# holo-routing/holo

Measured on AMD Instinct MI355X. Metric: full-SPF runs/sec on 100k-vertex synthetic LSDB, higher is better.
Workload: dtype u32; 1 GPU; isis-100k: IS-IS L2 100000 routers / 1000000 directed entries, metrics U[1,100], 64 concurrent SPF roots per GPU per step (BASELINE.json configs[2]); n_vertices=100000, n_entries=1000000, mask_words=1, outputs=dist u32 + hops u16 + flags u16 + first-hop mask u64 per (root,vertex), in HBM, steps_in_flight=4, gather=none

## Files before the change

holo_amd/build.py:

```python
from __future__ import annotations

import os
import shutil
import subprocess

HERE = os.path.dirname(os.path.abspath(__file__))
CSRC = os.path.join(HERE, "csrc")
LIB = os.path.join(HERE, "libholo_spf_hip.so")
SOURCES = ["spf_capi.hip", "hub_sort.hip"]
DEPS = ["spf_capi.hip", "spf_kernels.hip.h", "spf_repair.hip.h", "spf_lfa.hip.h", "spf_rlfa.hip.h", "spf_tilfa.hip.h", "graph_build.hip.h", "spf_multi.hip.h", "hub_sort.hip", "hub_sort.h", os.path.join("..", "..", "include", "holo_spf_hip.h")]


def hipcc_path() -> str:
    for cand in (shutil.which("hipcc"), "/opt/rocm/bin/hipcc"):
        if cand and os.path.exists(cand):
            return cand
    raise RuntimeError("hipcc not found: cannot build libholo_spf_hip.so")


def needs_build() -> bool:
    if not os.path.exists(LIB):
        return True
    t = os.path.getmtime(LIB)
    return any(os.path.getmtime(os.path.join(CSRC, d)) > t for d in DEPS)


def build_lib(force: bool = False, verbose: bool = False) -> str:
    if not force and not needs_build():
        return LIB
    flags = ["--offload-arch=gfx950", "-O3", "-std=c++17", "-fPIC", "-Wall", "-Wno-unused-function",
             "-mllvm", "-amdgpu-kernarg-preload-count=16"]
    flags += os.environ.get("HSPF_BUILD_DEFS", "").split()
    objs, procs = [], []
# ... 31 lines not shown
```

holo_amd/csrc/spf_capi.hip:

```cpp
#include "../../include/holo_spf_hip.h"
#include "spf_kernels.hip.h"
#include "spf_repair.hip.h"
#include "graph_build.hip.h"
#include "graph_patch.hip.h"
#include "hub_sort.h"
#include "spf_lfa.hip.h"
#include "spf_rlfa.hip.h"
#include "spf_tilfa.hip.h"

#include <algorithm>
#include <chrono>
#include <cstdio>
#include <cstdlib>
#include <cstring>
#include <atomic>
#include <condition_variable>
#include <deque>
#include <functional>
#include <mutex>
#include <thread>
#include <new>
#include <string>
#include <vector>

using namespace hspf;

namespace {

// ... 123 lines not shown
    g.out_ptr = d_out_ptr; g.out_dst = d_out_dst; g.out_w = d_out_w; g.out_fpos = d_out_fpos;
    for (int x = 0; x < 9; ++x) g.xcd_start[x] = xcd_start[x];
    g.unit_first = n_heavy_chunks ? d_unit_first : nullptr;
    g.n_heavy_units = n_heavy_chunks * 4u;
    for (int x = 0; x < 9; ++x) g.xcd_heavy[x] = xcd_heavy(x);
    g.giant_vtx = d_giant; g.giant_slice0 = d_giant + n_giant; g.n_giant = n_giant;
    return g;
  }
};

struct hspf_ctx {
  int device = 0;
  hipStream_t stream = nullptr;
  bool own_stream = true;
  std::string last_error;
  hipEvent_t ev[7] = {};
  DevBuf dist, hv, mask, lane_flags, changed, st64, stamp, hnb, kcnt, swcnt;
  uint32_t lean_head = 4, lean_passes = 16;
  uint32_t lean_dense_pct = 30;
  uint32_t lean_stay_pct = 10;
  uint32_t lean_dense_passes = 16;
  uint32_t lean_max_passes = 48;
  uint32_t lean_multi_min_wgs = 4096;
  DevBuf o_dist, o_hops, o_flags, o_mask, o_rank;
  DevBuf o_pack, pk_flag;
  char *h_stage = nullptr;
  size_t h_stage_cap = 0;
  hipEvent_t ev_stage[2] = {};
  DevBuf ex_list, ex_heap, ex_pos;
  DevBuf rp_rank;
  DevBuf dyn_part;
  DevBuf rp_trace;
  DevBuf rp_z, rp_ord, rp_work, rp_status;
  uint32_t *h_rp = nullptr; size_t h_rp_cap = 0;
  uint32_t est_rp_rounds = 6;
  uint32_t est_rp = 10;
  DevBuf pf_ptr, pf_vtx, pf_met, pf_org;
  bool pf_shadow_ok = false;
  uint32_t pf_shadow_nv = 0, pf_res_np = 0, pf_res_ne = 0;
  const void *pf_res_ptr = nullptr, *pf_res_vtx = nullptr, *pf_res_met = nullptr;
  DevBuf pack;
  uint32_t last_diff_count = 0;
  DevBuf evs_scr, evs_rec;
  DevBuf rlfa_key;
  DevBuf tilfa_key, tilfa_tw;
  DevBuf lfa_tab, lfa_scal;
// ... 523 lines not shown
    case HSPF_E_INTERNAL: return "internal invariant violated";
    case HSPF_E_NO_PACKED: return "results do not fit packed words";
    default: return "unknown error";
  }
}

const char *hspf_last_error(const hspf_ctx *ctx) { return ctx ? ctx->last_error.c_str() : ""; }

int hspf_init(int device_ordinal, hspf_ctx **out) {
  if (!out) return HSPF_E_INVAL;
  *out = nullptr;
  int n = 0;
  if (hipGetDeviceCount(&n) != hipSuccess || n <= 0) return HSPF_E_NODEV;
  if (device_ordinal < 0 || device_ordinal >= n) return HSPF_E_NODEV;
  hspf_ctx *ctx = new (std::nothrow) hspf_ctx();
  if (!ctx) return HSPF_E_NOMEM;
  ctx->device = device_ordinal;
  if (const char *v = getenv("HSPF_VARIANT")) ctx->variant = (uint32_t)strtoul(v, nullptr, 0);
  if (const char *v = getenv("HSPF_SINGLE_MAX_N")) ctx->single_max_n = (uint32_t)strtoul(v, nullptr, 0);
  if (const char *v = getenv("HSPF_DENSE_PASSES")) ctx->lean_dense_passes = std::min<uint32_t>(std::max<uint32_t>((uint32_t)strtoul(v, nullptr, 0), 1u), 32u);
  if (const char *v = getenv("HSPF_DENSE_PCT")) ctx->lean_dense_pct = (uint32_t)strtoul(v, nullptr, 0);
  if (const char *v = getenv("HSPF_DENSE_STAY_PCT")) ctx->lean_stay_pct = (uint32_t)strtoul(v, nullptr, 0);
  if (const char *v = getenv("HSPF_DENSE_MIN_WGS")) ctx->lean_multi_min_wgs = (uint32_t)strtoul(v, nullptr, 0);
  if (const char *v = getenv("HSPF_LEAN_HEAD")) ctx->lean_head = std::min<uint32_t>((uint32_t)strtoul(v, nullptr, 0), 60u);
  if (const char *v = getenv("HSPF_LV_MAX_ROOTS")) ctx->lv_max_roots = (uint32_t)strtoul(v, nullptr, 0);
  if (const char *v = getenv("HSPF_LV_MIN_N")) ctx->lv_min_n = (uint32_t)strtoul(v, nullptr, 0);
  if (const char *v = getenv("HSPF_XCD_MAX_ROOTS")) ctx->xcd_max_roots = std::min<uint32_t>((uint32_t)strtoul(v, nullptr, 0), XCD_MAX_ROOTS);
  if (const char *v = getenv("HSPF_XCD_ALWAYS")) ctx->xcd_always = strtoul(v, nullptr, 0) != 0;
  if (const char *v = getenv("HSPF_XCD_SKEW")) ctx->xcd_skew = atoi(v) != 0;
  if (const char *v = getenv("HSPF_XCD_TIMEOUT_MS")) ctx->xcd_timeout_ms = (uint32_t)strtoul(v, nullptr, 0);
  if (const char *v = getenv("HSPF_XCD_ROW_COST")) ctx->xcd_row_cost = (uint32_t)strtoul(v, nullptr, 0);
  if (const char *v = getenv("HSPF_UNIT_HEAVY_DEG")) ctx->unit_heavy_deg = (uint32_t)strtoul(v, nullptr, 0);
  if (const char *v = getenv("HSPF_HUB_DEG")) ctx->hub_deg = (uint32_t)strtoul(v, nullptr, 0);
  if (const char *v = getenv("HSPF_TW_HOST_MAX")) ctx->tw_host_max = strtoull(v, nullptr, 0);
  if (const char *v = getenv("HSPF_PATCH_FULL")) ctx->patch_full = atoi(v) != 0;
  if (const char *v = getenv("HSPF_ASYNC_LANES")) ctx->lanes_cfg = std::min<uint32_t>(std::max<uint32_t>((uint32_t)strtoul(v, nullptr, 0), 1u), 8u);
  if (hipSetDevice(device_ordinal) != hipSuccess) { delete ctx; return HSPF_E_NODEV; }
  if (hipStreamCreateWithFlags(&ctx->stream, hipStreamNonBlocking) != hipSuccess) { delete ctx; return HSPF_E_HIP; }
  for (auto &e : ctx->ev)
    if (hipEventCreate(&e) != hipSuccess) { delete ctx; return HSPF_E_HIP; }
  if (hipHostMalloc((void **)&ctx->h_changed, sizeof(int) * 256, hipHostMallocDefault) != hipSuccess) { delete ctx; return HSPF_E_NOMEM; }
  ctx->h_changed_cap = 256;
  if (hipHostMalloc((void **)&ctx->h_info, sizeof(BuildInfo), hipHostMallocDefault) != hipSuccess) { hspf_shutdown(ctx); return HSPF_E_NOMEM; }
  *out = ctx;
  return HSPF_OK;
}
// ... 892 lines not shown
  d_changed = (int *)ctx->changed.p;
  gd = g->dev();
  tabs = SlotTabs{d_up + w_ptr, d_up + w_vtx, d_up + w_base};
  if (row_map) od.row_map = d_up + w_map;
  ignore_ovl = (run_flags & HSPF_RUN_IGNORE_OVERLOAD) ? 1u : 0u;
  net_nh = (run_flags & HSPF_RUN_NET_NEXTHOPS) ? 1u : 0u;
  return HSPF_OK;
}

int Run::upload_block() {
  {
    uint32_t *h = ctx->h_up + (ctx->h_up_sel ? ctx->h_up_cap / 8 : 0);
    const uint32_t *prev = ctx->h_up + (ctx->h_up_sel ? 0 : ctx->h_up_cap / 8);
    std::fill(h, h + up_bytes / 4, 0u);
    std::fill(h + w_roots, h + w_roots + L, HSPF_NO_ROOT);
    std::copy(roots, roots + n_roots, h + w_roots);
    std::copy(tab_ptr.begin(), tab_ptr.end(), h + w_ptr);
    std::copy(tab_vtx.begin(), tab_vtx.end(), h + w_vtx);
    std::copy(tab_base.begin(), tab_base.end(), h + w_base);
    for (uint32_t r = 0; r < L; ++r) h[w_map + r] = (row_map && r < n_roots) ? row_map[r] : r;
    const FusedGraph fg{gd, tabs, d_kcnt, giant ? (uint32_t *)ctx->giant_part.p : (uint32_t *)nullptr,
                        (g->n_zero_rows && !g->hopcount_like) ? (uint32_t *)ctx->dyn_part.p : (uint32_t *)nullptr, L};
    memcpy(h + w_fg, &fg, sizeof(FusedGraph));
    st.dbg[2] = (uint32_t)std::chrono::duration_cast<std::chrono::microseconds>(std::chrono::steady_clock::now() - t_entry).count();
    const bool same = ctx->up_valid && ctx->up_len == up_bytes && memcmp(h, prev, up_bytes) == 0;
    if (!same) {
      HIPCHK(ctx, hipMemcpyAsync(d_up, h, up_bytes, hipMemcpyHostToDevice, s));
      ctx->up_valid = true; ctx->up_len = up_bytes; ctx->h_up_sel ^= 1;
    }
  }
  return HSPF_OK;
}

int Run::init_state() {
  d_st = (uint64_t *)ctx->st64.p;
  d_stamp = (uint32_t *)ctx->stamp.p;
  use_fw = !fused && !(ctx->variant & 64u) && (!g->hopcount_like || W <= 4);
  defer = use_fw && g->n_leaf != 0 && g->max_path_metric != HSPF_DIST_INF && !g->hopcount_like && g->n_zero_rows == 0;
  HIPCHK(ctx, hipEventRecord(ctx->ev[0], s));
  if (fused) {
  } else if (defer) {
    HIPCHK(ctx, hipMemsetAsync(d_lf, 0, (size_t)L * 4, s));
    const dim3 ig((unsigned)std::min<size_t>((rows / 64 + 3) / 4, 8192));
    switch (W) {
      case 1: hipLaunchKernelGGL(k_init_fw_state<1>, ig, dim3(256), 0, s, n, B, (const uint8_t *)g->d_leaf, d_dist, d_hv, d_mask); break;
      case 2: hipLaunchKernelGGL(k_init_fw_state<2>, ig, dim3(256), 0, s, n, B, (const uint8_t *)g->d_leaf, d_dist, d_hv, d_mask); break;
      case 4: hipLaunchKernelGGL(k_init_fw_state<4>, ig, dim3(256), 0, s, n, B, (const uint8_t *)g->d_leaf, d_dist, d_hv, d_mask); break;
// ... 117 lines not shown
      const bool zrows = dyn_parts;
      if (use_lean && zrows) st.dbg[0] |= 2u;
      if (dyn_parts && hipMemsetAsync(ctx->dyn_part.p, 0, (size_t)DYN_PARTS * L * 4, s) != hipSuccess) { ctx->last_error = "dyn partials"; return HSPF_E_HIP; }
      if (nar) hipLaunchKernelGGL((k_init_fused<uint32_t>), dim3((L + 3) / 4), dim3(256), 0, s, gd, (uint32_t *)d_st, d_stamp, (uint8_t *)ctx->hnb.p, d_roots, tabs, L, ns);
      else     hipLaunchKernelGGL((k_init_fused<uint64_t>), dim3((L + 3) / 4), dim3(256), 0, s, gd, d_st, d_stamp, (uint8_t *)ctx->hnb.p, d_roots, tabs, L, ns);
      uint32_t n_f = 0;
      const bool maxinf = g->max_path_metric == HSPF_DIST_INF;
      const bool plan_on = use_lean && !(ctx->variant & 524288u);
      const bool multi = ctx->lean_dense_passes > 1u && (uint64_t)fgrid.x * B >= ctx->lean_multi_min_wgs;
      const uint32_t per_launch = multi ? (uint32_t)std::min<uint64_t>(ctx->lean_dense_passes, ((1ull << 31) - 1u) / ((uint64_t)fgrid.x * B)) : 1u;
      const uint32_t plan_h = plan_on ? std::min(ctx->lean_head, 60u) : 0u;
      const uint32_t plan_P = plan_on ? std::min(std::max(ctx->lean_passes, 2u), std::min(ctx->lean_max_passes, 62u)) : 0u;
      const uint32_t plan_nd = plan_on ? (plan_P + per_launch - 1u) / per_launch : 0u;
      const uint64_t all_rows = (uint64_t)n * B;
      const uint32_t thr_enter = (uint32_t)std::min<uint64_t>(0xFFFFFFF0u, std::max<uint64_t>(1u, all_rows * ctx->lean_dense_pct / (100u * LEAN_SAMPLE)));
      const uint32_t thr_stay = ctx->lean_stay_pct == 0u ? 0u : (uint32_t)std::min<uint64_t>(0xFFFFFFF0u, std::max<uint64_t>(1u, all_rows * ctx->lean_stay_pct / (100u * LEAN_SAMPLE)));
      if (use_lean) {
        int e2 = ensure(ctx, ctx->swcnt, LEAN_CTL_WORDS * 4, false);
        if (e2) return e2;
      }
      uint32_t *d_ctl = (uint32_t *)ctx->swcnt.p;
      if (plan_on) ctx->est_fused = std::max(ctx->est_fused, plan_h + plan_nd + (ctx->est_seen ? 2u : 13u));
      ctx->est_seen = true;
      rb_ctl = plan_on ? d_ctl : nullptr;
      int r2 = run_phase(ctx->est_fused, pre_zeroed, [&](uint32_t sweep) {
#define HSPF_LAUNCH_FUSED2(ST_, MI_, CN_, UN_, stp_) hipLaunchKernelGGL((k_fused<ST_, MI_, CN_, UN_>), fgrid, dim3(256), 0, s, d_fg, d_changed, (int)sweep, d_stamp, (const uint8_t *)ctx->hnb.p, n, gd.in_ptr, gd.out_ptr, gd.vflags, stp_, d_roots, d_lf, net_nh, ignore_ovl, P, gd.in_src, gd.in_w, gd.out_dst, gd.e_in)
#define HSPF_LAUNCH_FUSED(ST_, MI_, CN_, stp_) do { if (units) HSPF_LAUNCH_FUSED2(ST_, MI_, CN_, true, stp_); else HSPF_LAUNCH_FUSED2(ST_, MI_, CN_, false, stp_); } while (0)
        const bool units = g->n_heavy_chunks != 0;
        if (use_lean) {
#define HSPF_LAUNCH_LEAN3(CN_, MD_, HD_, BM_, ZR_, grid_, pgr_, base_, thr_) hipLaunchKernelGGL((k_fused_lean<CN_, MD_, HD_, BM_, ZR_>), grid_, dim3(256), 0, s, d_fg, d_changed, (int)sweep, d_stamp, (const uint8_t *)ctx->hnb.p, n, (const uint32_t *)g->d_ell_so, (const uint32_t *)g->d_ell_w, (uint32_t *)d_st, (const uint32_t *)g->d_ell_od, d_roots, d_lf, net_nh, ignore_ovl, P, d_ctl, B, pgr_, base_, thr_)
#define HSPF_LAUNCH_LEAN2(CN_, MD_, HD_, BM_, grid_, pgr_, base_, thr_) do { if (zrows) HSPF_LAUNCH_LEAN3(CN_, MD_, HD_, BM_, true, grid_, pgr_, base_, thr_); else HSPF_LAUNCH_LEAN3(CN_, MD_, HD_, BM_, false, grid_, pgr_, base_, thr_); } while (0)
#define HSPF_LAUNCH_LEAN_C(MD_, HD_, grid_, pgr_, base_, thr_) do { if (count_rows) HSPF_LAUNCH_LEAN2(true, MD_, HD_, false, grid_, pgr_, base_, thr_); else HSPF_LAUNCH_LEAN2(false, MD_, HD_, false, grid_, pgr_, base_, thr_); } while (0)
#define HSPF_LAUNCH_LEAN_B(MD_, HD_, grid_, pgr_, base_, thr_) do { if (count_rows) HSPF_LAUNCH_LEAN2(true, MD_, HD_, true, grid_, pgr_, base_, thr_); else HSPF_LAUNCH_LEAN2(false, MD_, HD_, true, grid_, pgr_, base_, thr_); } while (0)
          const uint32_t bm_blocks = (n + (uint32_t)FVPB - 1u) / (uint32_t)FVPB;
          const bool bmaj = B >= 8u && 8ull * ((B + 7u) / 8u) * bm_blocks * per_launch < (1ull << 31);
          const dim3 bgrid(8u * ((B + 7u) / 8u) * bm_blocks);
          const PassGrid pg0{};
          if (sweep < plan_h) HSPF_LAUNCH_LEAN_C(0, true, fgrid, pg0, 0u, thr_enter);
          else if (sweep < plan_h + plan_nd) {
            const uint32_t base = (sweep - plan_h) * per_launch, np = std::min(per_launch, plan_P - base);
            if (bmaj) HSPF_LAUNCH_LEAN_B(1, false, dim3(bgrid.x * np), pass_grid(bgrid.x, bm_blocks), base, thr_stay);
            else      HSPF_LAUNCH_LEAN_C(1, false, dim3(fgrid.x * B * np), pass_grid(fgrid.x * B, fgrid.x), base, thr_stay);
          } else if (plan_on && sweep == plan_h + plan_nd) HSPF_LAUNCH_LEAN_C(2, false, fgrid, pg0, 0u, 0u);
          else HSPF_LAUNCH_LEAN_C(0, false, fgrid, pg0, 0u, 0u);
#undef HSPF_LAUNCH_LEAN_C
#undef HSPF_LAUNCH_LEAN_B
#undef HSPF_LAUNCH_LEAN2
#undef HSPF_LAUNCH_LEAN3
          return;
        }
        if (giant) {
          const dim3 ggrid(g->n_giant_slices, B);
#define HSPF_LAUNCH_GIANT(ST_, MI_, stp_) do { if (P.hc) hipLaunchKernelGGL((k_giant_part<ST_, MI_, true>), ggrid, dim3(256), 0, s, d_fg, (const int *)d_changed, (int)sweep, (const uint32_t *)d_stamp, n, (const ST_ *)stp_, (const uint32_t *)d_roots, net_nh, ignore_ovl, P); \
                                            else hipLaunchKernelGGL((k_giant_part<ST_, MI_, false>), ggrid, dim3(256), 0, s, d_fg, (const int *)d_changed, (int)sweep, (const uint32_t *)d_stamp, n, (const ST_ *)stp_, (const uint32_t *)d_roots, net_nh, ignore_ovl, P); } while (0)
          if (nar)         HSPF_LAUNCH_GIANT(uint32_t, false, (uint32_t *)d_st);
          else if (maxinf) HSPF_LAUNCH_GIANT(uint64_t, true, d_st);
          else             HSPF_LAUNCH_GIANT(uint64_t, false, d_st);
#undef HSPF_LAUNCH_GIANT
        }
        if (count_rows) {
          if (nar)         HSPF_LAUNCH_FUSED(uint32_t, false, true, (uint32_t *)d_st);
// ... 2 lines not shown
        } else {
          if (nar)         HSPF_LAUNCH_FUSED(uint32_t, false, false, (uint32_t *)d_st);
          else if (maxinf) HSPF_LAUNCH_FUSED(uint64_t, true, false, d_st);
          else             HSPF_LAUNCH_FUSED(uint64_t, false, false, d_st);
        }
#undef HSPF_LAUNCH_FUSED2
#undef HSPF_LAUNCH_FUSED
      }, n_f, [&]() {
        (void)hipEventRecord(ctx->ev[2], s);
        if (dyn_parts) hipLaunchKernelGGL(k_lf_reduce, dim3((L + 255) / 256), dim3(256), 0, s, d_lf, (const uint32_t *)ctx->dyn_part.p, L);
        const int rg = spec_fill ? (int)chunk_last : -1;
        emit_reset = rg >= 0;
        if (nar) hipLaunchKernelGGL((k_emit_fused<uint32_t>), dim3((n + 63) / 64, B), dim3(256), 0, s, n, n_roots, (uint32_t *)d_st, P, ode, ns, use_lean ? d_lf : (uint32_t *)nullptr, (const int *)d_changed, rg, fillw);
        else     hipLaunchKernelGGL((k_emit_fused<uint64_t>), dim3((n + 63) / 64, B), dim3(256), 0, s, n, n_roots, d_st, P, ode, ns, (uint32_t *)nullptr, (const int *)d_changed, rg, fillw);
        (void)hipEventRecord(ctx->ev[4], s);
        tail_done = true;
      });
      spec_fill = nullptr;
      if (r2) return r2;
      if (spec_done) ctx->prefill = hspf_ctx::Prefill{true, g->build_id, n, B, (uint32_t)esz, spec_nz, L, true, ns, fillw};
      ctx->est_fused = n_f + 1;
      st.n_relax_launches += n_f;
      if (count_rows) for (uint32_t i = 0; i < 256; ++i) st.rows_recomputed += ctx->h_lane_flags[L + i];
      if (plan_on) {
        const uint32_t *hc = ctx->h_lane_flags + L + 256;
        uint32_t trig = plan_h;
        for (uint32_t k = 0; k < plan_h; ++k) if (hc[LEAN_CTL_DUE + k * LEAN_CTL_STRIDE] == LEAN_SENTINEL) { trig = k; break; }
        uint32_t used = 0;
        for (uint32_t k = 0; k < plan_P; ++k) if (hc[LEAN_CTL_PCH + k * LEAN_CTL_STRIDE] != 0u) used = k + 1u;
        st.dbg[1] = (used & 0xFFu) | ((trig & 0xFFu) << 8) | ((plan_P & 0xFFu) << 16) | ((plan_h & 0x7Fu) << 24);
        const bool last_triggers = plan_h != 0u && hc[LEAN_CTL_DUE + (plan_h - 1u) * LEAN_CTL_STRIDE] != LEAN_SENTINEL && hc[LEAN_CTL_DUE + (plan_h - 1u) * LEAN_CTL_STRIDE] >= thr_enter;
        if (trig < plan_h) ctx->lean_head = std::max(trig, 1u);
        else if (plan_h != 0u && !last_triggers && used >= 2u) ctx->lean_head = std::min(plan_h + 1u, 60u);
        ctx->lean_passes = used >= plan_P ? std::min(ctx->lean_max_passes, plan_P + plan_P / 2u + 1u) : std::max(used + 1u, 2u);
      }
      return HSPF_OK;
    }

int Run::lv_run() {
      int r2;
      if ((r2 = ensure(ctx, ctx->stamp, (size_t)n_roots * n * 4))) return r2;
      uint32_t *a_stamp = (uint32_t *)ctx->stamp.p;
      hipError_t er = hipMemsetAsync(d_lf, 0, (size_t)L * 4, s);
      if (er == hipSuccess) er = hipMemsetAsync(d_st, 0xFF, (size_t)n_roots * n * 8, s);
      if (er == hipSuccess) er = hipMemsetAsync(a_stamp, 0, (size_t)n_roots * n * 4, s);
      if (er == hipSuccess && count_rows) er = hipMemsetAsync(d_kcnt, 0, 256 * 4, s);
// ... 725 lines not shown
    for (int c = 0; c < 3; ++c) {
      const uint32_t off = start[c], nr = start[c + 1] - start[c];
      if (nr == 0 || c == last_cls) continue;
      hspf_lane::Job job{g, std::vector<uint32_t>(proots.begin() + off, proots.begin() + off + nr), run_flags, U, 0,
                         std::vector<uint32_t>(dest.begin() + off, dest.begin() + off + nr), n_roots};
      cls_ticket[c] = lane_submit(ctx, std::move(job));
    }
  int rc_first = HSPF_OK;
  for (int c = 2; c >= 0; --c) {
    const uint32_t off = start[c], nr = start[c + 1] - start[c];
    if (nr == 0) continue;
    hspf_stats lane_st{};
    if (cls_ticket[c]) rc = lane_collect(ctx, cls_ticket[c], &lane_st);
    else rc = run_impl(ctx, g, proots.data() + off, nr, run_flags, &U, false, dest.data() + off, n_roots);
    if (rc) { if (!rc_first) rc_first = rc; continue; }
    const hspf_stats &p = cls_ticket[c] ? lane_st : ctx->stats;
    acc.n_roots += p.n_roots; acc.n_batches += p.n_batches; acc.n_relax_launches += p.n_relax_launches;
    acc.n_dag_launches += p.n_dag_launches; acc.n_exact_roots += p.n_exact_roots; acc.n_repaired_roots += p.n_repaired_roots; acc.repair_sweeps = std::max(acc.repair_sweeps, p.repair_sweeps); acc.repair_evals += p.repair_evals; acc.repair_groups += p.repair_groups; acc.ms_repair += p.ms_repair;
    acc.n_mask_words = std::max(acc.n_mask_words, p.n_mask_words);
    acc.ms_total += p.ms_total; acc.ms_relax += p.ms_relax; acc.ms_dag += p.ms_dag; acc.ms_finish += p.ms_finish;
    acc.state_bytes = std::max(acc.state_bytes, p.state_bytes); acc.narrow_overflow += p.narrow_overflow;
    acc.rows_recomputed += p.rows_recomputed;
    acc.dbg[0] |= p.dbg[0]; acc.dbg[1] = ((acc.dbg[1] | p.dbg[1]) & 0x80000000u) | ((acc.dbg[1] & 0x7FFFFFFFu) + (p.dbg[1] & 0x7FFFFFFFu));
    acc.dbg[2] += p.dbg[2]; acc.dbg[3] += p.dbg[3];
  }
  if (rc_first) return rc_first;
  if (!leaf_jobs.empty()) {
    const auto t_leaf = std::chrono::steady_clock::now();
    (void)hipSetDevice(ctx->device);
    if ((rc = ensure(ctx, ctx->leaf_jobs, leaf_jobs.size() * sizeof(LeafRootJob), false))) return rc;
    HIPCHK(ctx, hipMemcpyAsync(ctx->leaf_jobs.p, leaf_jobs.data(), leaf_jobs.size() * sizeof(LeafRootJob), hipMemcpyHostToDevice, s));
    hipLaunchKernelGGL(k_leaf_root_rows, dim3((n + 255u) / 256u, (uint32_t)leaf_jobs.size()), dim3(256), 0, s, n,
                       (const LeafRootJob *)ctx->leaf_jobs.p, (const uint32_t *)g->d_row_ptr[g->cur], (const uint32_t *)g->d_metric[g->cur], g->max_path_metric, W, U.dist, U.hops,
                       U.vflags_out, U.first_hop_mask);
    HIPCHK(ctx, hipGetLastError());
    HIPCHK(ctx, hipStreamSynchronize(s));
    acc.n_roots += (uint32_t)leaf_jobs.size();
    const float ms = std::chrono::duration<float, std::milli>(std::chrono::steady_clock::now() - t_leaf).count();
    acc.ms_total += ms; acc.ms_finish += ms;
  }
  if (side_by_side) {
    const float wall = std::chrono::duration<float, std::milli>(std::chrono::steady_clock::now() - t_cls).count();
    if (wall < acc.ms_total) {
      const float k = wall / acc.ms_total;
      acc.ms_total = wall; acc.ms_relax *= k; acc.ms_dag *= k; acc.ms_finish *= k;
    }
  }
// ... 87 lines not shown
}

int hspf_get_stats(const hspf_ctx *ctx, hspf_stats *out) {
  if (!ctx || !out) return HSPF_E_INVAL;
  *out = ctx->stats;
  return HSPF_OK;
}


static int lanes_ensure(hspf_ctx *ctx) {
  if (!ctx->lanes.empty()) return HSPF_OK;
  if (ctx->parent) { ctx->last_error = "asynchronous runs on a lane context"; return HSPF_E_INVAL; }
  (void)hipSetDevice(ctx->device);
  for (uint32_t i = 0; i < ctx->lanes_cfg; ++i) {
    hspf_lane *ln = new (std::nothrow) hspf_lane();
    if (!ln) { lanes_shutdown(ctx); return HSPF_E_NOMEM; }
    int rc = hspf_init(ctx->device, &ln->sub);
    if (rc == HSPF_OK) {
      hspf_ctx *c = ln->sub;
      c->parent = ctx;
      c->variant = ctx->variant; c->single_max_n = ctx->single_max_n; c->lv_max_roots = ctx->lv_max_roots; c->lv_min_n = ctx->lv_min_n; c->xcd_max_roots = ctx->xcd_max_roots; c->xcd_timeout_ms = ctx->xcd_timeout_ms; c->xcd_skew = ctx->xcd_skew; c->xcd_always = ctx->xcd_always;
      c->lean_dense_pct = ctx->lean_dense_pct; c->lean_stay_pct = ctx->lean_stay_pct; c->lean_dense_passes = ctx->lean_dense_passes;
      c->lean_head = ctx->lean_head; c->lean_passes = ctx->lean_passes; c->hub_deg = ctx->hub_deg; c->lean_multi_min_wgs = ctx->lean_multi_min_wgs;
      c->unit_heavy_deg = ctx->unit_heavy_deg; c->xcd_row_cost = ctx->xcd_row_cost;
    }
    if (rc != HSPF_OK) { if (ln->sub) hspf_shutdown(ln->sub); delete ln; lanes_shutdown(ctx); ctx->last_error = "could not create a lane context"; return rc; }
    for (auto &e : ln->stage_ev) if (hipEventCreateWithFlags(&e, hipEventDisableTiming) != hipSuccess) e = nullptr;
    if (!ctx->copy_stream && hipStreamCreateWithFlags(&ctx->copy_stream, hipStreamNonBlocking) != hipSuccess) ctx->copy_stream = nullptr;
    ctx->lanes.push_back(ln);
    ln->th = std::thread([ln, nl = ctx->lanes_cfg]() {
      for (;;) {
        std::unique_lock<std::mutex> lk(ln->mu);
        ln->cv.wait(lk, [&] { return !ln->jobs.empty() || ln->quit; });
        if (ln->jobs.empty()) return;
        hspf_lane::Job job = std::move(ln->jobs.front());
        ln->jobs.pop_front();
        ln->running = true;
        lk.unlock();
        ln->cv.notify_all();
        (void)hipSetDevice(ln->sub->device);
        hipEvent_t job_copy_ev = nullptr;
        const int rc = guarded(ln->sub, [&]() {
          if (job.packed) {
            hspf_ctx *par = ln->sub->parent;
            const size_t need = (size_t)8 * job.roots.size() * job.g->n;
            const uint64_t max_pairs = 1ull << 26;
// ... 815 lines not shown
```

holo_amd/csrc/spf_kernels.hip.h:

```cpp
#pragma once
#include <hip/hip_runtime.h>
#include <stdint.h>
#include <type_traits>

namespace hspf {

constexpr uint32_t INF = 0xFFFFFFFFu;
constexpr uint32_t SRC_NO_TRANSIT = 0x80000000u;
constexpr uint32_t SRC_LEAF = 0x40000000u;
constexpr uint32_t SRC_MASK = 0x3FFFFFFFu;

constexpr uint32_t HV_EPOCH_SHIFT = 16;
constexpr uint32_t HV_EPOCH_MAX = 0xFFFFu;

constexpr uint32_t LF_NEED_EXACT = 1u;
constexpr uint32_t LF_OVERFLOW = 2u;
constexpr uint32_t LF_DYN = 4u;

constexpr int WAVES_PER_BLOCK = 4;
constexpr int VPW = 4;
constexpr int VPB = WAVES_PER_BLOCK * VPW;

struct GraphDev {
  uint32_t n;
// ... 1095 lines not shown
  const uint32_t bx = bmaj ? (fpass >> 3) - fq * pgr.blocks : (MODE == 1 ? fpass - fq * pgr.blocks : blockIdx.x);
  const uint32_t pg = MODE == 1 ? pass_base + pidx : 0u;
  uint32_t pc2 = LEAN_SENTINEL, pc3 = LEAN_SENTINEL;
  if (MODE == 1 && thr != 0u && pg >= 2u && pg < 64u) {
    pc2 = ctl[LEAN_CTL_PCH + (pg - 2u) * LEAN_CTL_STRIDE];
    if (pg >= 3u) pc3 = ctl[LEAN_CTL_PCH + (pg - 3u) * LEAN_CTL_STRIDE];
  }
  const bool sampler = wave == 0u && (bmaj ? (bx & 7u) == 0u : ((bx >> 3) & 7u) == 0u);
  const uint32_t chunk = bmaj ? bx : xcd_chunk(gp->g.xcd_start, bx);
  if (MODE == 1 && min(pc2, pc3) < thr) {
    if (bx == 0u && batch == 0u && threadIdx.x == 0) changed[sweep] = 1;
    return;
  }
  if (chunk == 0xFFFFFFFFu || (bmaj && batch >= nbat)) return;
  const uint32_t wbeg = chunk * (uint32_t)FVPB + wave * (uint32_t)FVPW;
  if (wbeg >= n) return;
  uint32_t *A = act + (size_t)batch * n;
  const uint32_t cur = (uint32_t)sweep + 2u;
  const uint32_t vl = min(wbeg + min(lane, (uint32_t)VPW - 1u), n - 1);
  const uint32_t av = MODE == 0 ? A[vl] : cur;
  const uint32_t hb = hnb[(size_t)batch * n + vl] & (ignore_ovl ? ~RF_NT : ~0u);
  const uint32_t due4 = (uint32_t)__ballot(lane < (uint32_t)VPW && wbeg + lane < n && av >= cur);
  if (MODE == 0 && due4 == 0u) return;
  if (HEAD && sampler && lane == 0 && (uint32_t)sweep < 64u) atomicAdd(&ctl[LEAN_CTL_DUE + (uint32_t)sweep * LEAN_CTL_STRIDE], (uint32_t)__builtin_popcount(due4));
  ST *S = st + (size_t)batch * (n + 1u) * 64;
  const __amdgpu_buffer_rsrc_t rs = st_rsrc(S, (n + 1u) << 8);
  const uint32_t lane4 = lane * 4u;
  uint32_t sov[VPW], wk[VPW], od[VPW], oldq[VPW];
#pragma unroll
  for (int i = 0; i < VPW; ++i) {
    const uint32_t e = (min(wbeg + i, n) * 16u + (lane & 15u)) * 4u;
    sov[i] = *(const uint32_t *)((const char *)ell_so + e);
    wk[i] = *(const uint32_t *)((const char *)ell_w + e);
    od[i] = MODE == 1 ? 0u : *(const uint32_t *)((const char *)ell_od + e);
    oldq[i] = __builtin_amdgcn_raw_buffer_load_b32(rs, lane4, min(wbeg + i, n - 1) << 8, 0);
  }
  const uint32_t fast4 = (uint32_t)__ballot(lane < (uint32_t)VPW && hb == 0u) & due4;
  const uint32_t fasth4 = (uint32_t)__ballot(lane < (uint32_t)VPW && (hb & ~RF_ROOT) == RF_HNB) & due4;
  const uint32_t fastz4 = (!ZROWS || P.hc) ? 0u : ((uint32_t)__ballot(lane < (uint32_t)VPW && hb == RF_ZERO) & due4);
  const uint32_t root_slot = batch * 64 + lane;
  const __amdgpu_buffer_rsrc_t ra = st_rsrc(A, n * 4u);
  uint32_t info[VPW];
#pragma unroll
  for (int i = 0; i < VPW; ++i) {
    info[i] = rdlane(sov[i], 0) & 0xFFu;
    sov[i] &= ~0xFFu;
    wk[i] = (wk[i] << P.sh) + ((lane & 7u) << (P.sh - 3u));
    od[i] = lane < 16u ? od[i] : 0xFFFFFFFFu;
  }
  uint64_t any = 0ull;
  bool dyn = false;
  uint32_t n_done = 0, n_chg = 0;
  lean_group<COUNT, MODE, ZROWS>(gp, rs, ra, lane, lane4, wbeg, cur, P, roots, root_slot, net_nexthops, ignore_ovl, due4, fast4, fasth4, fastz4,
                          sov, wk, od, oldq, info, any, dyn, n_done, n_chg);
  if (MODE == 1) { if (bx == 0u && batch == 0u && threadIdx.x == 0) changed[sweep] = 1; }
  else if (any != 0ull && lane == 0) changed[sweep] = 1;
  if (COUNT && lane == 0) atomicAdd(&gp->rows_done[(blockIdx.x + wave) & 255u], n_done);
  if (MODE == 1 && sampler && lane == 0 && n_chg != 0u && pg < 64u) atomicAdd(&ctl[LEAN_CTL_PCH + pg * LEAN_CTL_STRIDE], n_chg);
  if (ZROWS && dyn) raise_dyn(gp, lane_flags, root_slot, blockIdx.x * 4u + wave);
}

constexpr int SINGLE_THREADS = 1024;
constexpr uint32_t SINGLE_MAX_N = 8192;
constexpr uint32_t SINGLE_MAX_E = 65536;
constexpr size_t SINGLE_LDS_MAX = 160 * 1024 - 64;

__device__ __forceinline__ void single_store_flags(uint32_t *lane_flags, uint32_t root_slot, uint32_t lf, int *word) {
  __syncthreads();
  if (threadIdx.x == 0) *word = 0;
  __syncthreads();
  if (lf) atomicOr(word, (int)lf);
  __syncthreads();
  if (threadIdx.x == 0) lane_flags[root_slot] = (uint32_t)*word;
}

struct SingleArgs {
  const FusedGraph *gp;
  const uint32_t *roots;
  FusedParams P;
  uint32_t net_nexthops, ignore_ovl, n_roots, count_rows, lds_links;
  uint32_t *lane_flags;
// ... 1866 lines not shown
```

Before: 157,700 spf_runs/s.

## Add compacting scan kernel for sparse lean sweeps with learned per-sweep plan

Adds k_lean_scan, where each block first ballots due and fast-path bits for 16 chunks of vertices, then has its four waves work only through the groups that have due rows. This cuts the wave launches and idle waves that the lean kernel spends on sparse sweeps. A host-side plan records per-sweep due counts from the sampler and picks the scan kernel on later runs for sweeps whose count falls below a threshold. The sampler atomic now fires in all MODE 0 launches, and the debug counters are packed, which adds some atomics and a different grid shape.

```diff
diff --git a/holo_amd/build.py b/holo_amd/build.py
--- a/holo_amd/build.py
+++ b/holo_amd/build.py
@@ -8,7 +8,7 @@
 CSRC = os.path.join(HERE, "csrc")
 LIB = os.path.join(HERE, "libholo_spf_hip.so")
 SOURCES = ["spf_capi.hip", "hub_sort.hip"]
-DEPS = ["spf_capi.hip", "spf_kernels.hip.h", "spf_repair.hip.h", "spf_lfa.hip.h", "spf_rlfa.hip.h", "spf_tilfa.hip.h", "graph_build.hip.h", "spf_multi.hip.h", "hub_sort.hip", "hub_sort.h", os.path.join("..", "..", "include", "holo_spf_hip.h")]
+DEPS = ["spf_capi.hip", "spf_kernels.hip.h", "spf_repair.hip.h", "spf_lfa.hip.h", "spf_rlfa.hip.h", "spf_tilfa.hip.h", "graph_build.hip.h", "spf_multi.hip.h", "hub_sort.hip", "hub_sort.h", "lean_scan_plan.h", os.path.join("..", "..", "include", "holo_spf_hip.h")]
 
 
 def hipcc_path() -> str:
diff --git a/holo_amd/csrc/lean_scan_plan.h b/holo_amd/csrc/lean_scan_plan.h
--- /dev/null
+++ b/holo_amd/csrc/lean_scan_plan.h
@@ -0,0 +1,27 @@
+#pragma once
+#include <cstdint>
+
+namespace hspf {
+
+struct LeanScanPlan {
+  uint64_t sparse = 0;
+  uint32_t from = 0xFFFFFFFFu;
+  bool takes(uint32_t k) const { return k >= from || (k < 64u && ((sparse >> k) & 1ull) != 0ull); }
+};
+
+constexpr uint32_t LEAN_SCAN_NOT_STAMPED = 0xFFFFFFFFu;
+
+inline LeanScanPlan lean_scan_learn(const uint32_t *counts, uint32_t n_seen, uint32_t thr) {
+  LeanScanPlan p;
+  p.from = n_seen;
+  for (uint32_t k = 0; k < n_seen && k < 64u; ++k)
+    if (counts[k] < thr) p.sparse |= 1ull << k;
+  return p;
+}
+
+inline uint32_t lean_scan_threshold(uint64_t all_rows, uint32_t pct, uint32_t sample) {
+  const uint64_t t = all_rows * pct / (100ull * sample);
+  return (uint32_t)(t < 1u ? 1u : (t > 0xFFFFFFF0ull ? 0xFFFFFFF0ull : t));
+}
+
+}
diff --git a/holo_amd/csrc/spf_capi.hip b/holo_amd/csrc/spf_capi.hip
--- a/holo_amd/csrc/spf_capi.hip
+++ b/holo_amd/csrc/spf_capi.hip
@@ -4,6 +4,7 @@
 #include "graph_build.hip.h"
 #include "graph_patch.hip.h"
 #include "hub_sort.h"
+#include "lean_scan_plan.h"
 #include "spf_lfa.hip.h"
 #include "spf_rlfa.hip.h"
 #include "spf_tilfa.hip.h"
@@ -173,6 +174,9 @@
   uint32_t lean_dense_passes = 16;
   uint32_t lean_max_passes = 48;
   uint32_t lean_multi_min_wgs = 4096;
+  uint32_t lean_scan = 1;
+  uint32_t lean_scan_pct = 2;
+  LeanScanPlan lean_scan_plan;
   DevBuf o_dist, o_hops, o_flags, o_mask, o_rank;
   DevBuf o_pack, pk_flag;
   char *h_stage = nullptr;
@@ -742,6 +746,8 @@
   if (const char *v = getenv("HSPF_DENSE_PCT")) ctx->lean_dense_pct = (uint32_t)strtoul(v, nullptr, 0);
   if (const char *v = getenv("HSPF_DENSE_STAY_PCT")) ctx->lean_stay_pct = (uint32_t)strtoul(v, nullptr, 0);
   if (const char *v = getenv("HSPF_DENSE_MIN_WGS")) ctx->lean_multi_min_wgs = (uint32_t)strtoul(v, nullptr, 0);
+  if (const char *v = getenv("HSPF_LEAN_SCAN")) ctx->lean_scan = std::min<uint32_t>((uint32_t)strtoul(v, nullptr, 0), 2u);
+  if (const char *v = getenv("HSPF_LEAN_SCAN_PCT")) ctx->lean_scan_pct = (uint32_t)strtoul(v, nullptr, 0);
   if (const char *v = getenv("HSPF_LEAN_HEAD")) ctx->lean_head = std::min<uint32_t>((uint32_t)strtoul(v, nullptr, 0), 60u);
   if (const char *v = getenv("HSPF_LV_MAX_ROOTS")) ctx->lv_max_roots = (uint32_t)strtoul(v, nullptr, 0);
   if (const char *v = getenv("HSPF_LV_MIN_N")) ctx->lv_min_n = (uint32_t)strtoul(v, nullptr, 0);
@@ -1680,7 +1686,7 @@
     const FusedGraph fg{gd, tabs, d_kcnt, giant ? (uint32_t *)ctx->giant_part.p : (uint32_t *)nullptr,
                         (g->n_zero_rows && !g->hopcount_like) ? (uint32_t *)ctx->dyn_part.p : (uint32_t *)nullptr, L};
     memcpy(h + w_fg, &fg, sizeof(FusedGraph));
-    st.dbg[2] = (uint32_t)std::chrono::duration_cast<std::chrono::microseconds>(std::chrono::steady_clock::now() - t_entry).count();
+    st.dbg[2] = (uint32_t)std::min<uint64_t>(0xFFFFFFu, (uint64_t)std::chrono::duration_cast<std::chrono::microseconds>(std::chrono::steady_clock::now() - t_entry).count());
     const bool same = ctx->up_valid && ctx->up_len == up_bytes && memcmp(h, prev, up_bytes) == 0;
     if (!same) {
       HIPCHK(ctx, hipMemcpyAsync(d_up, h, up_bytes, hipMemcpyHostToDevice, s));
@@ -1844,7 +1850,12 @@
       uint32_t *d_ctl = (uint32_t *)ctx->swcnt.p;
       if (plan_on) ctx->est_fused = std::max(ctx->est_fused, plan_h + plan_nd + (ctx->est_seen ? 2u : 13u));
       ctx->est_seen = true;
-      rb_ctl = plan_on ? d_ctl : nullptr;
+      rb_ctl = use_lean ? d_ctl : nullptr;
+      uint32_t sblocks = 1;
+      for (int x = 0; x < 8; ++x) sblocks = std::max(sblocks, (g->xcd_start[x + 1] - g->xcd_start[x] + 15u) / 16u);
+      const dim3 sgrid(8u * sblocks, B);
+      const LeanScanPlan scan_plan = ctx->lean_scan_plan;
+      std::vector<uint32_t> scan_launched;
       int r2 = run_phase(ctx->est_fused, pre_zeroed, [&](uint32_t sweep) {
 #define HSPF_LAUNCH_FUSED2(ST_, MI_, CN_, UN_, stp_) hipLaunchKernelGGL((k_fused<ST_, MI_, CN_, UN_>), fgrid, dim3(256), 0, s, d_fg, d_changed, (int)sweep, d_stamp, (const uint8_t *)ctx->hnb.p, n, gd.in_ptr, gd.out_ptr, gd.vflags, stp_, d_roots, d_lf, net_nh, ignore_ovl, P, gd.in_src, gd.in_w, gd.out_dst, gd.e_in)
 #define HSPF_LAUNCH_FUSED(ST_, MI_, CN_, stp_) do { if (units) HSPF_LAUNCH_FUSED2(ST_, MI_, CN_, true, stp_); else HSPF_LAUNCH_FUSED2(ST_, MI_, CN_, false, stp_); } while (0)
@@ -1858,7 +1869,18 @@
           const bool bmaj = B >= 8u && 8ull * ((B + 7u) / 8u) * bm_blocks * per_launch < (1ull << 31);
           const dim3 bgrid(8u * ((B + 7u) / 8u) * bm_blocks);
           const PassGrid pg0{};
-          if (sweep < plan_h) HSPF_LAUNCH_LEAN_C(0, true, fgrid, pg0, 0u, thr_enter);
+          const bool stamped = sweep < plan_h || !plan_on || sweep > plan_h + plan_nd;
+          if (stamped && (ctx->lean_scan == 2u || (ctx->lean_scan == 1u && scan_plan.takes(sweep)))) {
+#define HSPF_LAUNCH_SCAN3(CN_, HD_, ZR_, thr_) hipLaunchKernelGGL((k_lean_scan<CN_, HD_, ZR_>), sgrid, dim3(256), 0, s, d_fg, d_changed, (int)sweep, d_stamp, (const uint8_t *)ctx->hnb.p, n, (const uint32_t *)g->d_ell_so, (const uint32_t *)g->d_ell_w, (uint32_t *)d_st, (const uint32_t *)g->d_ell_od, d_roots, d_lf, net_nh, ignore_ovl, P, d_ctl, thr_)
+#define HSPF_LAUNCH_SCAN2(CN_, HD_, thr_) do { if (zrows) HSPF_LAUNCH_SCAN3(CN_, HD_, true, thr_); else HSPF_LAUNCH_SCAN3(CN_, HD_, false, thr_); } while (0)
+#define HSPF_LAUNCH_SCAN(HD_, thr_) do { if (count_rows) HSPF_LAUNCH_SCAN2(true, HD_, thr_); else HSPF_LAUNCH_SCAN2(false, HD_, thr_); } while (0)
+            if (sweep < plan_h) HSPF_LAUNCH_SCAN(true, thr_enter); else HSPF_LAUNCH_SCAN(false, 0u);
+#undef HSPF_LAUNCH_SCAN
+#undef HSPF_LAUNCH_SCAN2
+#undef HSPF_LAUNCH_SCAN3
+            scan_launched.push_back(sweep);
+          }
+          else if (sweep < plan_h) HSPF_LAUNCH_LEAN_C(0, true, fgrid, pg0, 0u, thr_enter);
           else if (sweep < plan_h + plan_nd) {
             const uint32_t base = (sweep - plan_h) * per_launch, np = std::min(per_launch, plan_P - base);
             if (bmaj) HSPF_LAUNCH_LEAN_B(1, false, dim3(bgrid.x * np), pass_grid(bgrid.x, bm_blocks), base, thr_stay);
@@ -1907,6 +1929,19 @@
       ctx->est_fused = n_f + 1;
       st.n_relax_launches += n_f;
       if (count_rows) for (uint32_t i = 0; i < 256; ++i) st.rows_recomputed += ctx->h_lane_flags[L + i];
+      if (use_lean) {
+        uint32_t ns_scan = st.dbg[2] >> 24;
+        for (uint32_t k : scan_launched) if (k < n_f) ++ns_scan;
+        st.dbg[2] = (st.dbg[2] & 0xFFFFFFu) | (std::min(ns_scan, 255u) << 24);
+        const uint32_t *hc = ctx->h_lane_flags + L + 256;
+        uint32_t cnt[64];
+        const uint32_t seen = std::min(n_f, 64u);
+        for (uint32_t k = 0; k < seen; ++k) {
+          const bool stamped = k < plan_h || !plan_on || k > plan_h + plan_nd;
+          cnt[k] = stamped ? hc[LEAN_CTL_DUE + k * LEAN_CTL_STRIDE] : LEAN_SCAN_NOT_STAMPED;
+        }
+        ctx->lean_scan_plan = lean_scan_learn(cnt, n_f, lean_scan_threshold(all_rows, ctx->lean_scan_pct, LEAN_SAMPLE));
+      }
       if (plan_on) {
         const uint32_t *hc = ctx->h_lane_flags + L + 256;
         uint32_t trig = plan_h;
@@ -2678,7 +2713,8 @@
     acc.state_bytes = std::max(acc.state_bytes, p.state_bytes); acc.narrow_overflow += p.narrow_overflow;
     acc.rows_recomputed += p.rows_recomputed;
     acc.dbg[0] |= p.dbg[0]; acc.dbg[1] = ((acc.dbg[1] | p.dbg[1]) & 0x80000000u) | ((acc.dbg[1] & 0x7FFFFFFFu) + (p.dbg[1] & 0x7FFFFFFFu));
-    acc.dbg[2] += p.dbg[2]; acc.dbg[3] += p.dbg[3];
+    acc.dbg[2] = std::min<uint32_t>(0xFFFFFFu, (acc.dbg[2] & 0xFFFFFFu) + (p.dbg[2] & 0xFFFFFFu)) | (std::min<uint32_t>(255u, (acc.dbg[2] >> 24) + (p.dbg[2] >> 24)) << 24);
+    acc.dbg[3] += p.dbg[3];
   }
   if (rc_first) return rc_first;
   if (!leaf_jobs.empty()) {
@@ -2812,6 +2848,7 @@
       c->variant = ctx->variant; c->single_max_n = ctx->single_max_n; c->lv_max_roots = ctx->lv_max_roots; c->lv_min_n = ctx->lv_min_n; c->xcd_max_roots = ctx->xcd_max_roots; c->xcd_timeout_ms = ctx->xcd_timeout_ms; c->xcd_skew = ctx->xcd_skew; c->xcd_always = ctx->xcd_always;
       c->lean_dense_pct = ctx->lean_dense_pct; c->lean_stay_pct = ctx->lean_stay_pct; c->lean_dense_passes = ctx->lean_dense_passes;
       c->lean_head = ctx->lean_head; c->lean_passes = ctx->lean_passes; c->hub_deg = ctx->hub_deg; c->lean_multi_min_wgs = ctx->lean_multi_min_wgs;
+      c->lean_scan = ctx->lean_scan; c->lean_scan_pct = ctx->lean_scan_pct;
       c->unit_heavy_deg = ctx->unit_heavy_deg; c->xcd_row_cost = ctx->xcd_row_cost;
     }
     if (rc != HSPF_OK) { if (ln->sub) hspf_shutdown(ln->sub); delete ln; lanes_shutdown(ctx); ctx->last_error = "could not create a lane context"; return rc; }
diff --git a/holo_amd/csrc/spf_kernels.hip.h b/holo_amd/csrc/spf_kernels.hip.h
--- a/holo_amd/csrc/spf_kernels.hip.h
+++ b/holo_amd/csrc/spf_kernels.hip.h
@@ -1141,7 +1141,7 @@
   const uint32_t hb = hnb[(size_t)batch * n + vl] & (ignore_ovl ? ~RF_NT : ~0u);
   const uint32_t due4 = (uint32_t)__ballot(lane < (uint32_t)VPW && wbeg + lane < n && av >= cur);
   if (MODE == 0 && due4 == 0u) return;
-  if (HEAD && sampler && lane == 0 && (uint32_t)sweep < 64u) atomicAdd(&ctl[LEAN_CTL_DUE + (uint32_t)sweep * LEAN_CTL_STRIDE], (uint32_t)__builtin_popcount(due4));
+  if (MODE == 0 && sampler && lane == 0 && (uint32_t)sweep < 64u) atomicAdd(&ctl[LEAN_CTL_DUE + (uint32_t)sweep * LEAN_CTL_STRIDE], (uint32_t)__builtin_popcount(due4));
   ST *S = st + (size_t)batch * (n + 1u) * 64;
   const __amdgpu_buffer_rsrc_t rs = st_rsrc(S, (n + 1u) << 8);
   const uint32_t lane4 = lane * 4u;
@@ -1176,6 +1176,97 @@
   else if (any != 0ull && lane == 0) changed[sweep] = 1;
   if (COUNT && lane == 0) atomicAdd(&gp->rows_done[(blockIdx.x + wave) & 255u], n_done);
   if (MODE == 1 && sampler && lane == 0 && n_chg != 0u && pg < 64u) atomicAdd(&ctl[LEAN_CTL_PCH + pg * LEAN_CTL_STRIDE], n_chg);
+  if (ZROWS && dyn) raise_dyn(gp, lane_flags, root_slot, blockIdx.x * 4u + wave);
+}
+
+template <bool COUNT, bool HEAD, bool ZROWS>
+__global__ __launch_bounds__(256) __attribute__((amdgpu_num_sgpr(80))) void k_lean_scan(
+    const FusedGraph *__restrict__ gp, int *changed, int sweep, uint32_t *__restrict__ act,
+    const uint8_t *__restrict__ hnb, uint32_t n_arg, const uint32_t *__restrict__ ell_so, const uint32_t *__restrict__ ell_w,
+    uint32_t *__restrict__ st, const uint32_t *__restrict__ ell_od, const uint32_t *__restrict__ roots, uint32_t *lane_flags,
+    uint32_t net_nexthops, uint32_t ignore_ovl, FusedParams P, uint32_t *__restrict__ ctl, uint32_t thr) {
+  typedef uint32_t ST;
+  if (sweep > 0 && changed[sweep - 1] == 0) return;
+  if (HEAD && sweep > 0 && ctl[LEAN_CTL_DUE + ((uint32_t)sweep - 1u) * LEAN_CTL_STRIDE] >= thr) {
+    if (blockIdx.x == 0 && blockIdx.y == 0 && threadIdx.x == 0) { ctl[LEAN_CTL_DUE + (uint32_t)sweep * LEAN_CTL_STRIDE] = LEAN_SENTINEL; changed[sweep] = 1; }
+    return;
+  }
+  __shared__ uint32_t s_bits[4][8];
+  __shared__ uint32_t s_grp[4];
+  const uint32_t lane = threadIdx.x & 63u;
+  const uint32_t wave = __builtin_amdgcn_readfirstlane(threadIdx.x >> 6);
+  const uint32_t batch = blockIdx.y, n = n_arg;
+  const uint32_t x = blockIdx.x & 7u, jb = blockIdx.x >> 3;
+  const uint32_t s0 = gp->g.xcd_start[x], s1 = gp->g.xcd_start[x + 1];
+  if (jb * 16u >= s1 - s0) return;
+  const uint32_t c0 = s0 + jb * 16u;
+  const uint32_t vbase = c0 * (uint32_t)FVPB, vend = min(min(c0 + 16u, s1) * (uint32_t)FVPB, n);
+  if (vbase >= n) return;
+  uint32_t *A = act + (size_t)batch * n;
+  const uint32_t cur = (uint32_t)sweep + 2u;
+  {
+    const uint32_t v = vbase + wave * 64u + lane, vl = min(v, n - 1u);
+    const uint32_t av = A[vl];
+    const uint32_t hb = hnb[(size_t)batch * n + vl] & (ignore_ovl ? ~RF_NT : ~0u);
+    const uint64_t due = __ballot(v < vend && av >= cur);
+    const uint64_t fast = __ballot(hb == 0u) & due;
+    const uint64_t fasth = __ballot((hb & ~RF_ROOT) == RF_HNB) & due;
+    const uint64_t fastz = (!ZROWS || P.hc) ? 0ull : (__ballot(hb == RF_ZERO) & due);
+    const uint32_t grp = (uint32_t)__ballot(lane < 16u && ((due >> ((lane & 15u) * 4u)) & 15ull) != 0ull);
+    if (lane == 0) {
+      s_bits[wave][0] = (uint32_t)due;   s_bits[wave][1] = (uint32_t)(due >> 32);
+      s_bits[wave][2] = (uint32_t)fast;  s_bits[wave][3] = (uint32_t)(fast >> 32);
+      s_bits[wave][4] = (uint32_t)fasth; s_bits[wave][5] = (uint32_t)(fasth >> 32);
+      s_bits[wave][6] = (uint32_t)fastz; s_bits[wave][7] = (uint32_t)(fastz >> 32);
+      s_grp[wave] = grp;
+      const uint32_t smp = (uint32_t)__builtin_popcount((uint32_t)due & 15u);
+      if ((wave & 1u) == 0u && smp != 0u && (uint32_t)sweep < 64u) atomicAdd(&ctl[LEAN_CTL_DUE + (uint32_t)sweep * LEAN_CTL_STRIDE], smp);
+    }
+  }
+  __syncthreads();
+  const uint32_t g01 = __builtin_amdgcn_readfirstlane(s_grp[0] | (s_grp[1] << 16));
+  const uint32_t g23 = __builtin_amdgcn_readfirstlane(s_grp[2] | (s_grp[3] << 16));
+  const uint64_t gmask = (uint64_t)g01 | ((uint64_t)g23 << 32);
+  if (gmask == 0ull) return;
+  ST *S = st + (size_t)batch * (n + 1u) * 64;
+  const __amdgpu_buffer_rsrc_t rs = st_rsrc(S, (n + 1u) << 8);
+  const __amdgpu_buffer_rsrc_t ra = st_rsrc(A, n * 4u);
+  const uint32_t lane4 = lane * 4u;
+  const uint32_t root_slot = batch * 64 + lane;
+  uint64_t any = 0ull;
+  bool dyn = false;
+  uint32_t n_done = 0, n_chg = 0, k = 0;
+#pragma unroll 1
+  for (uint64_t m = gmask; m != 0ull; m &= m - 1ull, ++k) {
+    if ((k & 3u) != wave) continue;
+    const uint32_t grp = (uint32_t)__builtin_ctzll(m);
+    const uint32_t sw = grp >> 4, half = (grp >> 3) & 1u, nib = (grp & 7u) * 4u;
+    const uint32_t due4 = (__builtin_amdgcn_readfirstlane(s_bits[sw][0 + half]) >> nib) & 15u;
+    const uint32_t fast4 = (__builtin_amdgcn_readfirstlane(s_bits[sw][2 + half]) >> nib) & 15u;
+    const uint32_t fasth4 = (__builtin_amdgcn_readfirstlane(s_bits[sw][4 + half]) >> nib) & 15u;
+    const uint32_t fastz4 = (!ZROWS || P.hc) ? 0u : ((__builtin_amdgcn_readfirstlane(s_bits[sw][6 + half]) >> nib) & 15u);
+    const uint32_t wbeg = vbase + grp * (uint32_t)VPW;
+    uint32_t sov[VPW], wk[VPW], od[VPW], oldq[VPW], info[VPW];
+#pragma unroll
+    for (int i = 0; i < VPW; ++i) {
+      const uint32_t e = (min(wbeg + i, n) * 16u + (lane & 15u)) * 4u;
+      sov[i] = *(const uint32_t *)((const char *)ell_so + e);
+      wk[i] = *(const uint32_t *)((const char *)ell_w + e);
+      od[i] = *(const uint32_t *)((const char *)ell_od + e);
+      oldq[i] = __builtin_amdgcn_raw_buffer_load_b32(rs, lane4, min(wbeg + i, n - 1) << 8, 0);
+    }
+#pragma unroll
+    for (int i = 0; i < VPW; ++i) {
+      info[i] = rdlane(sov[i], 0) & 0xFFu;
+      sov[i] &= ~0xFFu;
+      wk[i] = (wk[i] << P.sh) + ((lane & 7u) << (P.sh - 3u));
+      od[i] = lane < 16u ? od[i] : 0xFFFFFFFFu;
+    }
+    lean_group<COUNT, 0, ZROWS>(gp, rs, ra, lane, lane4, wbeg, cur, P, roots, root_slot, net_nexthops, ignore_ovl, due4, fast4, fasth4, fastz4,
+                                sov, wk, od, oldq, info, any, dyn, n_done, n_chg);
+  }
+  if (any != 0ull && lane == 0) changed[sweep] = 1;
+  if (COUNT && lane == 0 && n_done != 0u) atomicAdd(&gp->rows_done[(blockIdx.x + wave) & 255u], n_done);
   if (ZROWS && dyn) raise_dyn(gp, lane_flags, root_slot, blockIdx.x * 4u + wave);
 }
 
```

New measurement: 160,600 spf_runs/s (median of 6 runs). 1.02x the previous value.
